# ardaduz/deep-video-mvs

Measured on AMD Instinct MI355X. Metric: depth frames/sec/GPU @ 320x256x64 planes (fusionnet); rel-L1 vs ref, higher is better.
Workload: dtype f32

## Files before the change

deep-video-mvs_amd/csrc/direct_conv.hip:

```cpp
#include <stdlib.h>

#include "dvmvs_device.h"

namespace dvmvs {

typedef float float4v __attribute__((ext_vector_type(4)));

struct DirectConvArgs {
  const float* x;
  const float* packed;
  const float* bias;
  float* dst;
  float* dst_nhwc;
  long long x_batch_stride, dst_batch_stride;
  int B, C_in, C_out, H, W, OH, OW;
  int act;
  int n_groups;
  int packed_groups;
  int n_chunks;
  int tiles_x;
  int vec4;
};

#ifdef DVMVS_SWEEP_TRACE
// ... 343 lines not shown
    }
    const float* xb = x + static_cast<size_t>(b) * x_batch_stride;
#pragma unroll 2
    for (int c = c_lo; c < c_hi; ++c) {
      const float* plane = xb + static_cast<size_t>(c) * HW;
      float v[9];
#pragma unroll
      for (int t = 0; t < 9; ++t) v[t] = in[t] ? plane[off[t]] : 0.0f;
#pragma unroll
      for (int t = 0; t < 9; ++t) sum = fmaf(v[t], w[c * 9 + t], sum);
    }
  }
  s_part[slice][px] = sum;
  __syncthreads();
  if (slice == 0 && p < HW) {
    float total = s_part[0][px];
#pragma unroll
    for (int s = 1; s < SL; ++s) total += s_part[s][px];
    if (bias) total += bias[0];
    dst[static_cast<size_t>(b) * dst_batch_stride + p] = head_activation(total, act, p0, p1);
  }
}

struct DirectConvShape {
  int MW, MT, NT, PW, KS;
};
constexpr DirectConvShape kDcShapes[4] = {{16, 5, 2, 4, 2}, {8, 5, 2, 1, 8}, {16, 5, 1, 1, 8}, {8, 5, 1, 1, 8}};
constexpr int kDcCUs = 256;

inline int direct_conv_choose(int B, int C_in, int C_out, int H, int W, int K, int S) {
  if (B <= 0 || C_in <= 0 || C_out <= 0 || C_out % 16 != 0 || (K != 3 && K != 5) || (S != 1 && S != 2) || H <= 0 || W <= 0) return 0;
  if (S == 2 && (H % 2 != 0 || W % 2 != 0)) return 0;
  const int OH = H / S, OW = W / S;
#if defined(DVMVS_SWEEP_TUNING)
  const char* f = getenv("DVMVS_DC_SHAPE");
  const int forced = f ? atoi(f) : 0;
#else
  const int forced = 0;
#endif
  int best = 0;
  double best_fill = 0.0;
  for (int id = 1; id <= 4; ++id) {
    const DirectConvShape& s = kDcShapes[id - 1];
    const int tile_h = s.PW * (16 / s.MW), tile_w = s.MW * s.MT;
    if (OW % tile_w != 0 || C_out % (16 * s.NT) != 0) continue;
    if (forced == id) return id;
// ... 82 lines not shown
  const int id = direct_conv_choose(B, C_in, C_out, H, W, kernel_size, stride);
  if (id == 0) return DVMVS_EUNSUPPORTED;
  if (kDcShapes[id - 1].NT != n_tile) return DVMVS_EINVAL;
  DirectConvArgs a;
  a.x = x; a.packed = packed; a.bias = bias; a.dst = dst; a.dst_nhwc = dst_nhwc;
  a.B = B; a.C_in = C_in; a.C_out = C_out; a.H = H; a.W = W; a.OH = H / stride; a.OW = W / stride;
  a.x_batch_stride = x_batch_stride ? x_batch_stride : static_cast<long long>(C_in) * H * W;
  a.dst_batch_stride = dst_batch_stride ? dst_batch_stride : static_cast<long long>(C_out) * a.OH * a.OW;
  if (a.x_batch_stride < static_cast<long long>(C_in) * H * W || a.dst_batch_stride < static_cast<long long>(C_out) * a.OH * a.OW) return DVMVS_EINVAL;
  if (W % 4 != 0 || a.x_batch_stride % 4 != 0 || (reinterpret_cast<uintptr_t>(x) & 15) != 0) return DVMVS_EUNSUPPORTED;
  if (static_cast<long long>(C_in + 64) * H * W * 4 >= (1LL << 31)) return DVMVS_EUNSUPPORTED;
  a.act = activation;
  a.n_groups = (C_in + 3) / 4;
  a.packed_groups = dc_packed_groups(C_in);
  a.vec4 = (a.OW % 4 == 0 && (a.OH * a.OW) % 4 == 0 && a.dst_batch_stride % 4 == 0 && (reinterpret_cast<uintptr_t>(dst) & 15) == 0) ? 1 : 0;
  a.n_chunks = 0; a.tiles_x = 0;
  hipStream_t s = static_cast<hipStream_t>(stream);
  if (kernel_size == 3) return stride == 1 ? launch_direct_conv_shape<3, 1>(id, a, s) : launch_direct_conv_shape<3, 2>(id, a, s);
  return stride == 1 ? launch_direct_conv_shape<5, 1>(id, a, s) : launch_direct_conv_shape<5, 2>(id, a, s);
}

extern "C" int dvmvs_conv_head_fwd(const float* x, long long x_batch_stride, const float* weight, const float* bias, float* dst,
                                   long long dst_batch_stride, int B, int C_in, int H, int W, int activation, float p0, float p1, dvmvs_stream_t stream) {
  using namespace dvmvs;
  if (!x || !weight || !dst || B <= 0 || C_in <= 0 || H <= 0 || W <= 0) return DVMVS_EINVAL;
  if (activation < 0 || activation > 3) return DVMVS_EINVAL;
  const long long HW = static_cast<long long>(H) * W;
  if (x_batch_stride == 0) x_batch_stride = HW * C_in;
  if (dst_batch_stride == 0) dst_batch_stride = HW;
  hipStream_t s = static_cast<hipStream_t>(stream);
  if (HW >= 16384) {
    hipLaunchKernelGGL((conv_head_kernel<64>), dim3(static_cast<unsigned int>((HW + 63) / 64), B), dim3(256), 0, s, x, weight, bias, dst, x_batch_stride,
                       dst_batch_stride, C_in, H, W, activation, p0, p1);
  } else {
    hipLaunchKernelGGL((conv_head_kernel<16>), dim3(static_cast<unsigned int>((HW + 15) / 16), B), dim3(256), 0, s, x, weight, bias, dst, x_batch_stride,
                       dst_batch_stride, C_in, H, W, activation, p0, p1);
  }
  return launch_status();
}

#ifdef DVMVS_SWEEP_TRACE
extern "C" int dvmvs_debug_direct_conv_trace(unsigned long long* host, int waves) {
  if (waves > dvmvs::kDcTraceWaves) waves = dvmvs::kDcTraceWaves;
  return static_cast<int>(hipMemcpyFromSymbol(host, HIP_SYMBOL(dvmvs::g_dc_trace), sizeof(unsigned long long) * dvmvs::kDcTraceWords * waves));
}
#endif
```

deep-video-mvs_amd/csrc/frame_ops.hip:

```cpp
#include "dvmvs_device.h"

namespace dvmvs {

template <int ACT>
__device__ inline float apply_act(float v, float p0 = 0.0f, float p1 = 0.0f) {
  if (ACT == 1) return fmaxf(v, 0.0f);
  if (ACT == 2) return 1.0f / (1.0f + expf(-v));
  if (ACT == 3) {
#pragma clang fp contract(off)
    const float s = 1.0f / (1.0f + expf(-v));
    return 1.0f / (p0 * s + p1);
  }
  return v;
}

template <int ACT, bool VEC4, int RES>
__global__ __launch_bounds__(256) void bias_act_kernel(const float* x, float* dst, long long dst_batch_stride, const float* __restrict__ bias,
                                                       const float* __restrict__ residual, int C, int HW, int W, float p0, float p1) {
  const int plane = blockIdx.y;
  const int b = plane / C, c = plane - b * C;
  const float bv = bias ? bias[c] : 0.0f;
  const float* p = x + static_cast<size_t>(plane) * HW;
  float* d = dst + static_cast<size_t>(b) * dst_batch_stride + static_cast<size_t>(c) * HW;
  if (VEC4 && RES != 2) {
    typedef float float4v __attribute__((ext_vector_type(4)));
    const float4v* p4 = reinterpret_cast<const float4v*>(p);
    float4v* d4 = reinterpret_cast<float4v*>(d);
    const float4v* r4 = reinterpret_cast<const float4v*>(residual + (RES == 1 ? static_cast<size_t>(plane) * HW : 0));
    const int n4 = HW / 4;
    for (int i = blockIdx.x * blockDim.x + threadIdx.x; i < n4; i += gridDim.x * blockDim.x) {
      float4v v = p4[i];
#pragma unroll
      for (int e = 0; e < 4; ++e) v[e] = apply_act<ACT>(v[e] + bv, p0, p1);
      if (RES == 1) {
        const float4v r = r4[i];
#pragma unroll
        for (int e = 0; e < 4; ++e) v[e] += r[e];
      }
      d4[i] = v;
    }
  } else {
    const int Wh = W / 2;
    const float* r = RES == 1 ? residual + static_cast<size_t>(plane) * HW
                              : (RES == 2 ? residual + static_cast<size_t>(plane) * (HW / 4) : nullptr);
    for (int i = blockIdx.x * blockDim.x + threadIdx.x; i < HW; i += gridDim.x * blockDim.x) {
      float v = apply_act<ACT>(p[i] + bv, p0, p1);
      if (RES == 1) v += r[i];
      if (RES == 2) {
// ... 13 lines not shown
  const float sh = OH > 1 ? static_cast<float>(H - 1) / static_cast<float>(OH - 1) : 0.0f;
  const float sw = OW > 1 ? static_cast<float>(W - 1) / static_cast<float>(OW - 1) : 0.0f;
  const long long total = static_cast<long long>(planes) * OH * OW;
  for (long long i = blockIdx.x * static_cast<long long>(blockDim.x) + threadIdx.x; i < total;
       i += static_cast<long long>(gridDim.x) * blockDim.x) {
    const int ox = static_cast<int>(i % OW);
    const int oy = static_cast<int>((i / OW) % OH);
    const long long pl = i / (static_cast<long long>(OW) * OH);
    const float fy = sh * static_cast<float>(oy), fx = sw * static_cast<float>(ox);
    const int y0 = static_cast<int>(fy), x0 = static_cast<int>(fx);
    const int y1 = y0 + (y0 < H - 1 ? 1 : 0), x1 = x0 + (x0 < W - 1 ? 1 : 0);
    const float h1 = fy - static_cast<float>(y0), h0 = 1.0f - h1;
    const float w1 = fx - static_cast<float>(x0), w0 = 1.0f - w1;
    const float* p = in + pl * H * W;
    const long long b = pl / C, c = pl - b * C;
    const float bv = (PRE != 0 && pre_bias) ? pre_bias[c] : 0.0f;
    const float v00 = PRE ? apply_act<PRE>(p[y0 * W + x0] + bv) : p[y0 * W + x0], v01 = PRE ? apply_act<PRE>(p[y0 * W + x1] + bv) : p[y0 * W + x1];
    const float v10 = PRE ? apply_act<PRE>(p[y1 * W + x0] + bv) : p[y1 * W + x0], v11 = PRE ? apply_act<PRE>(p[y1 * W + x1] + bv) : p[y1 * W + x1];
    out[b * out_batch_stride + (c * OH + oy) * OW + ox] = h0 * (w0 * v00 + w1 * v01) + h1 * (w0 * v10 + w1 * v11);
  }
}

template <int PRE>
__device__ inline void upsample2x_quads_plane(const float* __restrict__ in, float* __restrict__ out, long long out_batch_stride, const float* __restrict__ pre_bias,
                                              int pl, int C, int H, int W) {
#pragma clang fp contract(off)
  typedef float float4v __attribute__((ext_vector_type(4)));
  const int OH = 2 * H, OW = 2 * W, QW = OW >> 2;
  const float sh = OH > 1 ? static_cast<float>(H - 1) / static_cast<float>(OH - 1) : 0.0f;
  const float sw = OW > 1 ? static_cast<float>(W - 1) / static_cast<float>(OW - 1) : 0.0f;
  const int b = pl / C, c = pl - b * C;
  const float* p = in + static_cast<size_t>(pl) * H * W;
  const float bv = (PRE != 0 && pre_bias) ? pre_bias[c] : 0.0f;
  float* dst = out + static_cast<size_t>(b) * out_batch_stride + static_cast<size_t>(c) * OH * OW;
  for (int q = blockIdx.x * 256 + threadIdx.x; q < OH * QW; q += gridDim.x * 256) {
    const int oy = q / QW, ox = 4 * (q - oy * QW);
    const float fy = sh * static_cast<float>(oy);
    const int y0 = static_cast<int>(fy);
    const int y1 = y0 + (y0 < H - 1 ? 1 : 0);
    const float h1 = fy - static_cast<float>(y0), h0 = 1.0f - h1;
    const float* r0 = p + y0 * W;
    const float* r1 = p + y1 * W;
    float4v v;
#pragma unroll
    for (int e = 0; e < 4; ++e) {
      const float fx = sw * static_cast<float>(ox + e);
      const int x0 = static_cast<int>(fx);
      const int x1 = x0 + (x0 < W - 1 ? 1 : 0);
      const float w1 = fx - static_cast<float>(x0), w0 = 1.0f - w1;
      const float v00 = PRE ? apply_act<PRE>(r0[x0] + bv) : r0[x0], v01 = PRE ? apply_act<PRE>(r0[x1] + bv) : r0[x1];
      const float v10 = PRE ? apply_act<PRE>(r1[x0] + bv) : r1[x0], v11 = PRE ? apply_act<PRE>(r1[x1] + bv) : r1[x1];
      v[e] = h0 * (w0 * v00 + w1 * v01) + h1 * (w0 * v10 + w1 * v11);
    }
    *reinterpret_cast<float4v*>(dst + oy * OW + ox) = v;
  }
}

template <int PRE>
__global__ __launch_bounds__(256) void upsample2x_quads_kernel(const float* __restrict__ in, float* __restrict__ out, long long out_batch_stride,
                                                               const float* __restrict__ pre_bias, int C, int H, int W) {
  upsample2x_quads_plane<PRE>(in, out, out_batch_stride, pre_bias, blockIdx.y, C, H, W);
}

template <int PRE2>
__global__ __launch_bounds__(256) void upsample2x_pair_quads_kernel(const float* __restrict__ in1, float* __restrict__ out1, long long out1_batch_stride, int C1,
                                                                    const float* __restrict__ in2, float* __restrict__ out2, long long out2_batch_stride,
                                                                    const float* __restrict__ pre_bias2, int C2, int planes1, int H, int W) {
  const int pl = blockIdx.y;
  if (pl < planes1) upsample2x_quads_plane<0>(in1, out1, out1_batch_stride, nullptr, pl, C1, H, W);
  else upsample2x_quads_plane<PRE2>(in2, out2, out2_batch_stride, pre_bias2, pl - planes1, C2, H, W);
}

template <int K, int ACT, bool PRE>
__global__ __launch_bounds__(256) void depthwise_conv_kernel(const float* __restrict__ in, const float* __restrict__ weight,
                                                             const float* __restrict__ bias, const float* __restrict__ pre_bias,
                                                             float* __restrict__ out, int C, int H, int W, int OH, int OW, int stride) {
  const int c = blockIdx.y, b = blockIdx.z;
  const float* wk = weight + static_cast<size_t>(c) * K * K;
  const float* src = in + (static_cast<size_t>(b) * C + c) * H * W;
  float* dst = out + (static_cast<size_t>(b) * C + c) * OH * OW;
  const float bv = bias ? bias[c] : 0.0f;
  const float pv = (PRE && pre_bias) ? pre_bias[c] : 0.0f;
  for (int i = blockIdx.x * blockDim.x + threadIdx.x; i < OH * OW; i += gridDim.x * blockDim.x) {
    const int oy = i / OW, ox = i - oy * OW;
    const int y0 = oy * stride - K / 2, x0 = ox * stride - K / 2;
    float acc = 0.0f;
#pragma unroll
    for (int ky = 0; ky < K; ++ky) {
      const int y = y0 + ky;
      const bool yin = y >= 0 && y < H;
#pragma unroll
      for (int kx = 0; kx < K; ++kx) {
        const int x = x0 + kx;
// ... 76 lines not shown
  if (!x || !dst || B <= 0 || C <= 0 || H <= 0 || W <= 0) return DVMVS_EINVAL;
  if (residual_mode < 0 || residual_mode > 2 || (residual_mode != 0 && !residual)) return DVMVS_EINVAL;
  if (dst_batch_stride < static_cast<long long>(C) * H * W) return DVMVS_EINVAL;
  if (residual_mode == 2 && ((H & 1) || (W & 1))) return DVMVS_EUNSUPPORTED;
  if (static_cast<long long>(B) * C > 65535LL) return DVMVS_EUNSUPPORTED;
  hipStream_t s = static_cast<hipStream_t>(stream);
  switch (activation) {
    case 0: return launch_bias_act<0>(x, dst, dst_batch_stride, bias, residual, residual_mode, B, C, H, W, p0, p1, s);
    case 1: return launch_bias_act<1>(x, dst, dst_batch_stride, bias, residual, residual_mode, B, C, H, W, p0, p1, s);
    case 2: return launch_bias_act<2>(x, dst, dst_batch_stride, bias, residual, residual_mode, B, C, H, W, p0, p1, s);
    case 3: return launch_bias_act<3>(x, dst, dst_batch_stride, bias, residual, residual_mode, B, C, H, W, p0, p1, s);
    default: return DVMVS_EINVAL;
  }
}

extern "C" int dvmvs_bias_act_inplace(float* x, const float* bias, const float* residual, int residual_mode, int B, int C, int H,
                                      int W, int activation, dvmvs_stream_t stream) {
  if (activation == 3) return DVMVS_EINVAL;
  return dvmvs_bias_act_fwd(x, x, static_cast<long long>(C) * H * W, bias, residual, residual_mode, B, C, H, W, activation, 0.0f, 0.0f, stream);
}

extern "C" int dvmvs_upsample2x_fwd(const float* in, float* out, long long out_batch_stride, const float* pre_bias, int pre_activation,
                                    int B, int C, int H, int W, dvmvs_stream_t stream) {
  using namespace dvmvs;
  if (!in || !out || B <= 0 || C <= 0 || H <= 0 || W <= 0) return DVMVS_EINVAL;
  if (pre_activation < 0 || pre_activation > 2) return DVMVS_EINVAL;
  if (out_batch_stride == 0) out_batch_stride = static_cast<long long>(C) * H * W * 4;
  if (out_batch_stride < static_cast<long long>(C) * H * W * 4) return DVMVS_EINVAL;
  const long long total = static_cast<long long>(B) * C * H * W * 4;
  long long blocks = (total + 255) / 256;
  if (blocks > 256LL * 16) blocks = 256LL * 16;
  const dim3 grid(static_cast<unsigned>(blocks)), block(256);
  hipStream_t s = static_cast<hipStream_t>(stream);
  if (W % 2 == 0 && (reinterpret_cast<uintptr_t>(out) & 15) == 0 && (out_batch_stride & 3) == 0 && static_cast<long long>(B) * C <= 65535 &&
      static_cast<long long>(H) * W < (1LL << 27)) {
    const int quads = 2 * H * (W / 2);
    const int per_plane = max(1, min((quads + 255) / 256, max(1, 4096 / (B * C))));
    const dim3 qgrid(static_cast<unsigned>(per_plane), static_cast<unsigned>(B * C));
    if (pre_activation == 1) hipLaunchKernelGGL(upsample2x_quads_kernel<1>, qgrid, block, 0, s, in, out, out_batch_stride, pre_bias, C, H, W);
    else if (pre_activation == 2) hipLaunchKernelGGL(upsample2x_quads_kernel<2>, qgrid, block, 0, s, in, out, out_batch_stride, pre_bias, C, H, W);
    else hipLaunchKernelGGL(upsample2x_quads_kernel<0>, qgrid, block, 0, s, in, out, out_batch_stride, pre_bias, C, H, W);
    return launch_status();
  }
  if (pre_activation == 1) hipLaunchKernelGGL(upsample2x_kernel<1>, grid, block, 0, s, in, out, out_batch_stride, pre_bias, B * C, C, H, W);
  else if (pre_activation == 2) hipLaunchKernelGGL(upsample2x_kernel<2>, grid, block, 0, s, in, out, out_batch_stride, pre_bias, B * C, C, H, W);
  else hipLaunchKernelGGL(upsample2x_kernel<0>, grid, block, 0, s, in, out, out_batch_stride, pre_bias, B * C, C, H, W);
  return launch_status();
}

extern "C" int dvmvs_upsample2x_pair_fwd(const float* in1, float* out1, long long out1_batch_stride, int C1, const float* in2, float* out2,
                                         long long out2_batch_stride, const float* pre_bias2, int pre_activation2, int C2, int B, int H, int W,
                                         dvmvs_stream_t stream) {
  using namespace dvmvs;
  if (!in1 || !out1 || !in2 || !out2 || B <= 0 || C1 <= 0 || C2 <= 0 || H <= 0 || W <= 0) return DVMVS_EINVAL;
  if (pre_activation2 < 0 || pre_activation2 > 2) return DVMVS_EINVAL;
  if (out1_batch_stride == 0) out1_batch_stride = static_cast<long long>(C1) * H * W * 4;
  if (out2_batch_stride == 0) out2_batch_stride = static_cast<long long>(C2) * H * W * 4;
  if (out1_batch_stride < static_cast<long long>(C1) * H * W * 4 || out2_batch_stride < static_cast<long long>(C2) * H * W * 4) return DVMVS_EINVAL;
  const long long planes = static_cast<long long>(B) * (C1 + C2);
  const bool quads = W % 2 == 0 && ((reinterpret_cast<uintptr_t>(out1) | reinterpret_cast<uintptr_t>(out2)) & 15) == 0 && ((out1_batch_stride | out2_batch_stride) & 3) == 0 &&
                     planes <= 65535 && static_cast<long long>(H) * W < (1LL << 27);
  if (!quads) {
    const int rc = dvmvs_upsample2x_fwd(in1, out1, out1_batch_stride, nullptr, 0, B, C1, H, W, stream);
    return rc != 0 ? rc : dvmvs_upsample2x_fwd(in2, out2, out2_batch_stride, pre_bias2, pre_activation2, B, C2, H, W, stream);
  }
  const int n_quads = 2 * H * (W / 2);
  const int per_plane = max(1, min((n_quads + 255) / 256, max(1, 4096 / static_cast<int>(planes))));
  const dim3 grid(static_cast<unsigned>(per_plane), static_cast<unsigned>(planes)), block(256);
  hipStream_t s = static_cast<hipStream_t>(stream);
#define DVMVS_UP2(P) hipLaunchKernelGGL(upsample2x_pair_quads_kernel<P>, grid, block, 0, s, in1, out1, out1_batch_stride, C1, in2, out2, out2_batch_stride, pre_bias2, C2, B * C1, H, W)
  if (pre_activation2 == 1) DVMVS_UP2(1); else if (pre_activation2 == 2) DVMVS_UP2(2); else DVMVS_UP2(0);
#undef DVMVS_UP2
  return launch_status();
}

extern "C" int dvmvs_depthwise_conv_fwd(const float* in, const float* weight, const float* bias, const float* pre_bias, int pre_relu,
                                        float* out, int B, int C, int H, int W, int kernel_size, int stride, int activation,
                                        dvmvs_stream_t stream) {
  using namespace dvmvs;
  if (!in || !weight || !out || B <= 0 || C <= 0 || H <= 0 || W <= 0) return DVMVS_EINVAL;
  if ((kernel_size != 3 && kernel_size != 5) || (stride != 1 && stride != 2) || activation < 0 || activation > 2) return DVMVS_EUNSUPPORTED;
  if (C > 65535 || B > 65535) return DVMVS_EUNSUPPORTED;
  const int pad = kernel_size / 2;
  const int OH = (H + 2 * pad - kernel_size) / stride + 1, OW = (W + 2 * pad - kernel_size) / stride + 1;
  hipStream_t s = static_cast<hipStream_t>(stream);
#define DVMVS_DW(K, A) return launch_depthwise<K, A>(in, weight, bias, pre_bias, pre_relu != 0, out, B, C, H, W, OH, OW, stride, s)
  if (kernel_size == 3) {
    if (activation == 0) DVMVS_DW(3, 0);
    if (activation == 1) DVMVS_DW(3, 1);
    DVMVS_DW(3, 2);
  }
  if (activation == 0) DVMVS_DW(5, 0);
  if (activation == 1) DVMVS_DW(5, 1);
  DVMVS_DW(5, 2);
// ... 31 lines not shown
```

deep-video-mvs_amd/dvmvs/hip/_capi.py:

```python
import ctypes
import os
import threading

import torch

_HERE = os.path.dirname(os.path.abspath(__file__))
LIB_PATH = os.environ.get("DVMVS_HIP_LIB", os.path.normpath(os.path.join(_HERE, "..", "..", "lib", "libdvmvs_hip.so")))

ABI_VERSION = 11
MAX_MEASUREMENTS = 8
MAX_DEPTH_LEVELS = 256
LAYOUT_NCHW, LAYOUT_NHWC = 0, 1

_c_fp = ctypes.c_void_p
_c_fpp = ctypes.POINTER(ctypes.c_void_p)
_c_int = ctypes.c_int
_c_dbl = ctypes.c_double
_c_stream = ctypes.c_void_p
_c_f3 = ctypes.POINTER(ctypes.c_float)

SIGNATURES = {
    "dvmvs_abi_version": (_c_int, []),
    "dvmvs_build_arch": (ctypes.c_char_p, []),
    "dvmvs_error_string": (ctypes.c_char_p, [_c_int]),
# ... 21 lines not shown
                                       _c_int, _c_int, _c_int, _c_int, _c_int, _c_int,
                                       _c_dbl, _c_dbl, _c_stream]),
    "dvmvs_hidden_warp_fwd": (_c_int, [_c_fp, _c_fp, _c_fp, _c_fp, _c_fp, _c_int, _c_int, _c_int, _c_int, _c_int, _c_stream]),
    "dvmvs_hidden_warp_bwd": (_c_int, [_c_fp, _c_fp, _c_fp, _c_fp, _c_fp, _c_int, _c_int, _c_int, _c_int, _c_stream]),
    "dvmvs_relative_pose": (_c_int, [_c_fp, _c_fp, _c_fp, _c_int, _c_stream]),
    "dvmvs_lstm_gates_fwd": (_c_int, [_c_fp, _c_fp, _c_fp, _c_fp, _c_int, _c_int, _c_int, _c_int, _c_stream]),
    "dvmvs_lstm_gates_bwd": (_c_int, [_c_fp, _c_fp, _c_fp, _c_fp, _c_fp, _c_fp, _c_int, _c_int, _c_int, _c_int, _c_stream]),
    "dvmvs_lstm_gates_partials_fwd": (_c_int, [_c_fp, _c_int, _c_fp, _c_fp, _c_fp, _c_int, _c_int, _c_int, _c_int, _c_stream]),
    "dvmvs_bottleneck_conv_packed_bytes": (ctypes.c_size_t, [_c_int, _c_int]),
    "dvmvs_bottleneck_conv_pack": (_c_int, [_c_fp, _c_fp, _c_int, _c_int, _c_stream]),
    "dvmvs_bottleneck_conv_splits": (_c_int, [_c_int] * 6),
    "dvmvs_bottleneck_conv_fwd": (_c_int, [_c_fp, _c_fp, _c_fp] + [_c_int] * 6 + [_c_stream]),
    "dvmvs_bottleneck_conv_up2x_fwd": (_c_int, [_c_fp, _c_fp, _c_fp] + [_c_int] * 5 + [_c_stream]),
    "dvmvs_direct_conv_tile": (_c_int, [_c_int] * 7),
    "dvmvs_direct_conv_packed_bytes": (ctypes.c_size_t, [_c_int] * 4),
    "dvmvs_direct_conv_pack": (_c_int, [_c_fp, _c_fp, _c_int, _c_int, _c_int, _c_int, _c_stream]),
    "dvmvs_direct_conv_fwd": (_c_int, [_c_fp, ctypes.c_longlong, _c_fp, _c_int, _c_fp, _c_fp, ctypes.c_longlong] + [_c_int] * 8 + [_c_stream]),
    "dvmvs_direct_conv_dual_fwd": (_c_int, [_c_fp, ctypes.c_longlong, _c_fp, _c_int, _c_fp, _c_fp, ctypes.c_longlong, _c_fp] + [_c_int] * 8 + [_c_stream]),
    "dvmvs_pointwise_conv_supported": (_c_int, [_c_int] * 7),
    "dvmvs_pointwise_conv_packed_bytes": (ctypes.c_size_t, [_c_int] * 2),
    "dvmvs_pointwise_conv_pack": (_c_int, [_c_fp, _c_fp, _c_int, _c_int, _c_stream]),
    "dvmvs_pointwise_conv_fwd": (_c_int, [_c_fp, ctypes.c_longlong, _c_fp, _c_fp, _c_fp, ctypes.c_longlong, _c_int, _c_fp, ctypes.c_longlong] + [_c_int] * 7 + [_c_stream]),
    "dvmvs_conv_head_fwd": (_c_int, [_c_fp, ctypes.c_longlong, _c_fp, _c_fp, _c_fp, ctypes.c_longlong] + [_c_int] * 5 + [ctypes.c_float, ctypes.c_float, _c_stream]),
    "dvmvs_partial_sums_bias_act_fwd": (_c_int, [_c_fp, _c_int, _c_fp, ctypes.c_longlong, _c_fp, _c_int, _c_int, _c_int, _c_int, _c_stream]),
    "dvmvs_depth_reproject_fwd": (_c_int, [_c_fp, _c_fp, _c_fp, _c_fp, _c_fp, _c_fp, _c_int,
                                           _c_int, _c_int, _c_int, _c_stream]),
    "dvmvs_bias_act_fwd": (_c_int, [_c_fp, _c_fp, ctypes.c_longlong, _c_fp, _c_fp, _c_int, _c_int, _c_int, _c_int, _c_int, _c_int,
                                    ctypes.c_float, ctypes.c_float, _c_stream]),
    "dvmvs_bias_act_inplace": (_c_int, [_c_fp, _c_fp, _c_fp, _c_int, _c_int, _c_int, _c_int, _c_int, _c_int, _c_stream]),
    "dvmvs_conv_bias_act_fwd": (_c_int, [_c_fp, _c_fp, _c_fp, _c_fp, ctypes.c_longlong] + [_c_int] * 9 + [_c_stream]),
    "dvmvs_upsample2x_fwd": (_c_int, [_c_fp, _c_fp, ctypes.c_longlong, _c_fp, _c_int, _c_int, _c_int, _c_int, _c_int, _c_stream]),
    "dvmvs_upsample2x_pair_fwd": (_c_int, [_c_fp, _c_fp, ctypes.c_longlong, _c_int, _c_fp, _c_fp, ctypes.c_longlong, _c_fp, _c_int, _c_int, _c_int, _c_int, _c_int, _c_stream]),
    "dvmvs_upsample2x_bwd": (_c_int, [_c_fp, _c_fp, _c_int, _c_int, _c_int, _c_int, _c_stream]),
    "dvmvs_depthwise_conv_bwd_workspace_bytes": (ctypes.c_size_t, [_c_int] * 6),
    "dvmvs_depthwise_conv_bwd": (_c_int, [_c_fp, _c_fp, _c_fp, _c_fp, _c_fp, _c_fp, _c_int, _c_int, _c_int, _c_int, _c_int, _c_int, _c_stream]),
    "dvmvs_depth_reproject_lowres_fwd": (_c_int, [_c_fp, _c_fp, _c_fp, _c_fp, _c_fp, _c_fp, _c_int, _c_int, _c_int, _c_int, _c_stream]),
    "dvmvs_depth_reproject_estimate_fwd": (_c_int, [_c_fp, _c_fp, _c_fp, _c_fp, _c_fp, _c_fp, _c_int, _c_int, _c_int, _c_int, _c_stream]),
    "dvmvs_tsdf_integrate": (_c_int, [_c_fp, _c_fp, _c_fp, _c_int, _c_int, _c_int, ctypes.c_float, ctypes.c_float, ctypes.c_float,
                                      ctypes.c_float, _c_fp, _c_fp, _c_fp, _c_fp, _c_int, _c_int, ctypes.c_float, ctypes.c_float, _c_stream]),
    "dvmvs_marching_cubes_workspace_bytes": (ctypes.c_size_t, [_c_int, _c_int, _c_int]),
    "dvmvs_marching_cubes_count": (_c_int, [_c_fp, _c_int, _c_int, _c_int, ctypes.c_float, _c_fp, ctypes.c_size_t, _c_fp, _c_stream]),
    "dvmvs_marching_cubes_emit": (_c_int, [_c_fp, _c_fp, _c_int, _c_int, _c_int, ctypes.c_float, ctypes.c_float, ctypes.c_float,
                                           ctypes.c_float, ctypes.c_float, _c_fp, _c_fp, _c_fp, _c_fp, _c_fp, ctypes.c_longlong,
                                           ctypes.c_longlong, _c_stream]),
    "dvmvs_depthwise_conv_fwd": (_c_int, [_c_fp, _c_fp, _c_fp, _c_fp, _c_int, _c_fp, _c_int, _c_int, _c_int, _c_int, _c_int, _c_int, _c_int,
                                          _c_stream]),
    "dvmvs_rgb_sweep_fwd": (_c_int, [_c_fp, _c_fpp, _c_fp, _c_fp, _c_fp, _c_int, _c_int, _c_int, _c_int, _c_int, _c_int,
                                     _c_dbl, _c_dbl, _c_int, _c_int, _c_int, _c_stream]),
    "dvmvs_gp_filter_step": (_c_int, [_c_fp, _c_fp, _c_fp, _c_int, _c_dbl, _c_dbl, _c_dbl, _c_dbl, _c_dbl, _c_dbl, _c_int, _c_stream]),
    "dvmvs_dps_volume_fwd": (_c_int, [_c_fp, _c_fp, _c_fp, _c_fp, _c_fp, _c_fp, _c_int, _c_int, _c_int, _c_int, _c_int, _c_dbl, _c_stream]),
    "dvmvs_dps_regress_fwd": (_c_int, [_c_fp, _c_fp, _c_fp, _c_int, _c_int, _c_int, _c_int, _c_int, _c_int, _c_dbl, _c_stream]),
    "dvmvs_preprocess_rgb_fwd": (_c_int, [_c_fp, _c_fp, _c_int, _c_int, _c_int, ctypes.c_longlong, _c_int, _c_int, _c_int, _c_int,
                                          ctypes.c_longlong, _c_dbl, _c_f3, _c_f3, _c_int, _c_stream]),
    "dvmvs_preprocess_depth_fwd": (_c_int, [_c_fp, _c_fp, _c_int, _c_int, _c_int, _c_int, _c_int, _c_int, _c_int, _c_dbl, _c_stream]),
}
# ... 50 lines not shown
```

include/dvmvs_hip.h:

```cpp
#ifndef DVMVS_HIP_H
#define DVMVS_HIP_H

#include <stddef.h>
#include <stdint.h>

#ifdef __cplusplus
extern "C" {
#endif

#define DVMVS_ABI_VERSION 11
#define DVMVS_MAX_MEASUREMENTS 8
#define DVMVS_MAX_DEPTH_LEVELS 256

#define DVMVS_LAYOUT_NCHW 0
#define DVMVS_LAYOUT_NHWC 1

#define DVMVS_EINVAL (-1)
#define DVMVS_EUNSUPPORTED (-2)
#define DVMVS_ELIBRARY (-3)

typedef void* dvmvs_stream_t;

int dvmvs_abi_version(void);
const char* dvmvs_build_arch(void);
// ... 62 lines not shown
size_t dvmvs_bottleneck_conv_packed_bytes(int C_out, int C_in);
int dvmvs_bottleneck_conv_pack(const float* weight, float* packed, int C_out, int C_in, dvmvs_stream_t stream);
int dvmvs_bottleneck_conv_splits(int B, int C_out, int C_in, int H_in, int W_in, int stride);
int dvmvs_bottleneck_conv_fwd(const float* x, const float* packed, float* partials, int B, int C_in, int H_in, int W_in, int C_out,
                              int stride, dvmvs_stream_t stream);
int dvmvs_bottleneck_conv_up2x_fwd(const float* x, const float* packed, float* partials, int B, int C_in, int H_in, int W_in, int C_out,
                                   dvmvs_stream_t stream);
int dvmvs_partial_sums_bias_act_fwd(const float* partials, int n_partials, float* dst, long long dst_batch_stride, const float* bias,
                                    int B, int C, int HW, int activation, dvmvs_stream_t stream);
int dvmvs_lstm_gates_partials_fwd(const float* conv_partials, int n_partials, const float* c_cur, float* h_next, float* c_next,
                                  int B, int hidden, int H, int W, dvmvs_stream_t stream);

int dvmvs_direct_conv_tile(int B, int C_in, int H, int W, int C_out, int kernel_size, int stride);
size_t dvmvs_direct_conv_packed_bytes(int C_out, int C_in, int kernel_size, int n_tile);
int dvmvs_direct_conv_pack(const float* weight, float* packed, int C_out, int C_in, int kernel_size, int n_tile, dvmvs_stream_t stream);
int dvmvs_direct_conv_fwd(const float* x, long long x_batch_stride, const float* packed, int n_tile, const float* bias, float* dst,
                          long long dst_batch_stride, int B, int C_in, int H, int W, int C_out, int kernel_size, int stride, int activation,
                          dvmvs_stream_t stream);
int dvmvs_direct_conv_dual_fwd(const float* x, long long x_batch_stride, const float* packed, int n_tile, const float* bias, float* dst,
                               long long dst_batch_stride, float* dst_nhwc, int B, int C_in, int H, int W, int C_out, int kernel_size, int stride,
                               int activation, dvmvs_stream_t stream);
int dvmvs_conv_head_fwd(const float* x, long long x_batch_stride, const float* weight, const float* bias, float* dst,
                        long long dst_batch_stride, int B, int C_in, int H, int W, int activation, float p0, float p1, dvmvs_stream_t stream);

int dvmvs_pointwise_conv_supported(int B, int C_in, int H, int W, int C_out, int activation, int residual_mode);
size_t dvmvs_pointwise_conv_packed_bytes(int C_out, int C_in);
int dvmvs_pointwise_conv_pack(const float* weight, float* packed, int C_out, int C_in, dvmvs_stream_t stream);
int dvmvs_pointwise_conv_fwd(const float* x, long long x_batch_stride, const float* packed, const float* bias, const float* residual,
                             long long residual_batch_stride, int residual_mode, float* dst, long long dst_batch_stride, int B, int C_in,
                             int H, int W, int C_out, int activation, int splits, dvmvs_stream_t stream);

int dvmvs_depth_reproject_fwd(const float* transformation, const float* previous_depth, const float* full_K,
                              const float* half_K, float* out, float* out_lowres, int lowres_factor,
                              int B, int full_height, int full_width, dvmvs_stream_t stream);
int dvmvs_depth_reproject_lowres_fwd(const float* transformation, const float* previous_depth, const float* full_K,
                                     const float* half_K, float* zbuffer, float* out_lowres, int lowres_factor,
                                     int B, int full_height, int full_width, dvmvs_stream_t stream);

int dvmvs_depth_reproject_estimate_fwd(const float* transformation, const float* previous_depth, const float* full_K,
                                       const float* half_K, float* estimate, float* estimate_to_clear, int lowres_factor,
                                       int B, int full_height, int full_width, dvmvs_stream_t stream);

int dvmvs_bias_act_fwd(const float* x, float* dst, long long dst_batch_stride, const float* bias, const float* residual,
                       int residual_mode, int B, int C, int H, int W, int activation, float p0, float p1, dvmvs_stream_t stream);
int dvmvs_bias_act_inplace(float* x, const float* bias, const float* residual, int residual_mode, int B, int C, int H, int W,
                           int activation, dvmvs_stream_t stream);
int dvmvs_upsample2x_fwd(const float* in, float* out, long long out_batch_stride, const float* pre_bias, int pre_activation,
                         int B, int C, int H, int W, dvmvs_stream_t stream);
int dvmvs_upsample2x_pair_fwd(const float* in1, float* out1, long long out1_batch_stride, int C1, const float* in2, float* out2,
                              long long out2_batch_stride, const float* pre_bias2, int pre_activation2, int C2, int B, int H, int W,
                              dvmvs_stream_t stream);
int dvmvs_conv_bias_act_fwd(const float* x, const float* weight, const float* bias, float* out, long long out_batch_stride,
                            int B, int Cin, int H, int W, int Cout, int K, int stride, int padding, int activation, dvmvs_stream_t stream);
int dvmvs_depthwise_conv_fwd(const float* in, const float* weight, const float* bias, const float* pre_bias, int pre_relu, float* out,
                             int B, int C, int H, int W, int kernel_size, int stride, int activation, dvmvs_stream_t stream);

int dvmvs_tsdf_integrate(float* tsdf_vol, float* weight_vol, float* color_vol, int dim_x, int dim_y, int dim_z,
                         float origin_x, float origin_y, float origin_z, float voxel_size, const float* cam_intr,
                         const float* cam_pose, const float* color_im, const float* depth_im, int im_h, int im_w,
                         float trunc_margin, float obs_weight, dvmvs_stream_t stream);

size_t dvmvs_marching_cubes_workspace_bytes(int X, int Y, int Z);
int dvmvs_marching_cubes_count(const float* vol, int X, int Y, int Z, float level, void* workspace, size_t workspace_bytes,
                               long long* counts_dev, dvmvs_stream_t stream);
int dvmvs_marching_cubes_emit(const float* vol, const float* color_vol, int X, int Y, int Z, float level, float ox, float oy, float oz,
                              float voxel_size, void* workspace, float* verts, float* normals, unsigned char* colors, int* faces,
                              long long V, long long F, dvmvs_stream_t stream);

int dvmvs_rgb_sweep_fwd(const float* image1, const float* const* image2s, const float* Hm, const float* kt, float* out,
                        int B, int M, int C, int H, int W, int D, double min_depth, double max_depth, int Cout,
                        int channel_offset, int copy_image, dvmvs_stream_t stream);
int dvmvs_gp_filter_step(double* state, const float* y, float* z, int N, double a00, double a01, double a10, double a11,
                         double k0, double k1, int reset, dvmvs_stream_t stream);

// ... 16 lines not shown
```

Before: 1410.

## Add register-blocked conv head and two-row bilinear upsample kernels as defaults

```diff
diff --git a/deep-video-mvs_amd/csrc/direct_conv.hip b/deep-video-mvs_amd/csrc/direct_conv.hip
--- a/deep-video-mvs_amd/csrc/direct_conv.hip
+++ b/deep-video-mvs_amd/csrc/direct_conv.hip
@@ -389,6 +389,85 @@
   }
 }
 
+template <int SL, int RUNS, bool VEC>
+__global__ __launch_bounds__(SL * RUNS) void conv_head_runs_kernel(const float* __restrict__ x, const float* __restrict__ w, const float* __restrict__ bias,
+                                                                   float* __restrict__ dst, long long x_batch_stride, long long dst_batch_stride, int C, int H,
+                                                                   int W, int act, float p0, float p1) {
+  constexpr int RUN = 4, CH = 8, NT = SL * RUNS;
+  __shared__ float s_part[SL][RUNS * RUN];
+  const int run = threadIdx.x % RUNS;
+  const int slice = RUNS % 64 == 0 ? __builtin_amdgcn_readfirstlane(threadIdx.x / RUNS) : threadIdx.x / RUNS;
+  const int HW = H * W, rpr = (W + RUN - 1) / RUN;
+  const int b = blockIdx.y;
+  const int g = blockIdx.x * RUNS + run;
+  const int y = g / rpr, x0 = (g - y * rpr) * RUN;
+  const int per = (C + SL - 1) / SL;
+  const int c_lo = slice * per, c_hi = min(C, c_lo + per);
+  float sum[RUN] = {0.0f, 0.0f, 0.0f, 0.0f};
+  if (y < H) {
+    bool rin[3], cin[RUN + 2];
+    int roff[3];
+#pragma unroll
+    for (int r = 0; r < 3; ++r) {
+      const int yy = y + r - 1;
+      rin[r] = yy >= 0 && yy < H;
+      roff[r] = rin[r] ? yy * W + x0 : x0;
+    }
+#pragma unroll
+    for (int j = 0; j < RUN + 2; ++j) cin[j] = x0 + j - 1 >= 0 && x0 + j - 1 < W;
+    const float* xb = x + static_cast<size_t>(b) * x_batch_stride;
+    for (int c0 = c_lo; c0 < c_hi; c0 += CH) {
+      float v[CH][3][RUN + 2];
+#pragma unroll
+      for (int k = 0; k < CH; ++k) {
+        if (c0 + k < c_hi) {
+          const float* plane = xb + static_cast<size_t>(c0 + k) * HW;
+#pragma unroll
+          for (int r = 0; r < 3; ++r) {
+            const float* row = plane + roff[r];
+            if (VEC) {
+              float4v q = {0.0f, 0.0f, 0.0f, 0.0f};
+              if (rin[r]) q = *reinterpret_cast<const float4v*>(row);
+#pragma unroll
+              for (int j = 0; j < RUN; ++j) v[k][r][j + 1] = q[j];
+            } else {
+#pragma unroll
+              for (int j = 1; j <= RUN; ++j) v[k][r][j] = (rin[r] && cin[j]) ? row[j - 1] : 0.0f;
+            }
+            v[k][r][0] = (rin[r] && cin[0]) ? row[-1] : 0.0f;
+            v[k][r][RUN + 1] = (rin[r] && cin[RUN + 1]) ? row[RUN] : 0.0f;
+          }
+        }
+      }
+#pragma unroll
+      for (int k = 0; k < CH; ++k) {
+        if (c0 + k < c_hi) {
+          const float* wc = w + (c0 + k) * 9;
+#pragma unroll
+          for (int e = 0; e < RUN; ++e) {
+#pragma unroll
+            for (int t = 0; t < 9; ++t) sum[e] = fmaf(v[k][t / 3][e + t % 3], wc[t], sum[e]);
+          }
+        }
+      }
+    }
+  }
+#pragma unroll
+  for (int e = 0; e < RUN; ++e) s_part[slice][run * RUN + e] = sum[e];
+  __syncthreads();
+  for (int j = threadIdx.x; j < RUNS * RUN; j += NT) {
+    const int gj = blockIdx.x * RUNS + j / RUN;
+    const int yj = gj / rpr, xj = (gj - yj * rpr) * RUN + j % RUN;
+    if (yj < H && xj < W) {
+      float total = s_part[0][j];
+#pragma unroll
+      for (int s = 1; s < SL; ++s) total += s_part[s][j];
+      if (bias) total += bias[0];
+      dst[static_cast<size_t>(b) * dst_batch_stride + yj * W + xj] = head_activation(total, act, p0, p1);
+    }
+  }
+}
+
 struct DirectConvShape {
   int MW, MT, NT, PW, KS;
 };
@@ -517,20 +596,37 @@
 
 extern "C" int dvmvs_conv_head_fwd(const float* x, long long x_batch_stride, const float* weight, const float* bias, float* dst,
                                    long long dst_batch_stride, int B, int C_in, int H, int W, int activation, float p0, float p1, dvmvs_stream_t stream) {
+  return dvmvs_conv_head_variant_fwd(x, x_batch_stride, weight, bias, dst, dst_batch_stride, B, C_in, H, W, activation, p0, p1, 0, stream);
+}
+
+extern "C" int dvmvs_conv_head_variant_fwd(const float* x, long long x_batch_stride, const float* weight, const float* bias, float* dst,
+                                           long long dst_batch_stride, int B, int C_in, int H, int W, int activation, float p0, float p1, int variant,
+                                           dvmvs_stream_t stream) {
   using namespace dvmvs;
   if (!x || !weight || !dst || B <= 0 || C_in <= 0 || H <= 0 || W <= 0) return DVMVS_EINVAL;
-  if (activation < 0 || activation > 3) return DVMVS_EINVAL;
+  if (activation < 0 || activation > 3 || variant < 0 || variant > 1) return DVMVS_EINVAL;
   const long long HW = static_cast<long long>(H) * W;
   if (x_batch_stride == 0) x_batch_stride = HW * C_in;
   if (dst_batch_stride == 0) dst_batch_stride = HW;
   hipStream_t s = static_cast<hipStream_t>(stream);
-  if (HW >= 16384) {
-    hipLaunchKernelGGL((conv_head_kernel<64>), dim3(static_cast<unsigned int>((HW + 63) / 64), B), dim3(256), 0, s, x, weight, bias, dst, x_batch_stride,
-                       dst_batch_stride, C_in, H, W, activation, p0, p1);
-  } else {
-    hipLaunchKernelGGL((conv_head_kernel<16>), dim3(static_cast<unsigned int>((HW + 15) / 16), B), dim3(256), 0, s, x, weight, bias, dst, x_batch_stride,
-                       dst_batch_stride, C_in, H, W, activation, p0, p1);
-  }
+  const bool large = HW >= 16384;
+  if (variant == 1) {
+    if (large) {
+      hipLaunchKernelGGL((conv_head_kernel<64>), dim3(static_cast<unsigned int>((HW + 63) / 64), B), dim3(256), 0, s, x, weight, bias, dst, x_batch_stride,
+                         dst_batch_stride, C_in, H, W, activation, p0, p1);
+    } else {
+      hipLaunchKernelGGL((conv_head_kernel<16>), dim3(static_cast<unsigned int>((HW + 15) / 16), B), dim3(256), 0, s, x, weight, bias, dst, x_batch_stride,
+                         dst_batch_stride, C_in, H, W, activation, p0, p1);
+    }
+    return launch_status();
+  }
+  const long long runs = static_cast<long long>(H) * ((W + 3) / 4);
+  const bool vec = W % 4 == 0 && x_batch_stride % 4 == 0 && (reinterpret_cast<uintptr_t>(x) & 15) == 0;
+#define DVMVS_HEAD(SL, RUNS, V) hipLaunchKernelGGL((conv_head_runs_kernel<SL, RUNS, V>), dim3(static_cast<unsigned int>((runs + RUNS - 1) / RUNS), B), dim3(SL * RUNS), \
+                                                   0, s, x, weight, bias, dst, x_batch_stride, dst_batch_stride, C_in, H, W, activation, p0, p1)
+  if (large) { if (vec) DVMVS_HEAD(4, 64, true); else DVMVS_HEAD(4, 64, false); }
+  else { if (vec) DVMVS_HEAD(16, 4, true); else DVMVS_HEAD(16, 4, false); }
+#undef DVMVS_HEAD
   return launch_status();
 }
 
diff --git a/deep-video-mvs_amd/csrc/frame_ops.hip b/deep-video-mvs_amd/csrc/frame_ops.hip
--- a/deep-video-mvs_amd/csrc/frame_ops.hip
+++ b/deep-video-mvs_amd/csrc/frame_ops.hip
@@ -1,6 +1,8 @@
 #include "dvmvs_device.h"
 
 namespace dvmvs {
+
+typedef float float4v __attribute__((ext_vector_type(4)));
 
 template <int ACT>
 __device__ inline float apply_act(float v, float p0 = 0.0f, float p1 = 0.0f) {
@@ -23,7 +25,6 @@
   const float* p = x + static_cast<size_t>(plane) * HW;
   float* d = dst + static_cast<size_t>(b) * dst_batch_stride + static_cast<size_t>(c) * HW;
   if (VEC4 && RES != 2) {
-    typedef float float4v __attribute__((ext_vector_type(4)));
     const float4v* p4 = reinterpret_cast<const float4v*>(p);
     float4v* d4 = reinterpret_cast<float4v*>(d);
     const float4v* r4 = reinterpret_cast<const float4v*>(residual + (RES == 1 ? static_cast<size_t>(plane) * HW : 0));
@@ -83,10 +84,34 @@
 }
 
 template <int PRE>
+__device__ inline float4v upsample2x_row_quad(const float* __restrict__ p, float bv, float sh, float sw, int oy, int ox, int H, int W) {
+#pragma clang fp contract(off)
+  const float fy = sh * static_cast<float>(oy);
+  const int y0 = static_cast<int>(fy);
+  const int y1 = y0 + (y0 < H - 1 ? 1 : 0);
+  const float h1 = fy - static_cast<float>(y0), h0 = 1.0f - h1;
+  const float* r0 = p + y0 * W;
+  const float* r1 = p + y1 * W;
+  float4v v;
+#pragma unroll
+  for (int e = 0; e < 4; ++e) {
+    const float fx = sw * static_cast<float>(ox + e);
+    const int x0 = static_cast<int>(fx);
+    const int x1 = x0 + (x0 < W - 1 ? 1 : 0);
+    const float w1 = fx - static_cast<float>(x0), w0 = 1.0f - w1;
+    const float v00 = PRE ? apply_act<PRE>(r0[x0] + bv) : r0[x0], v01 = PRE ? apply_act<PRE>(r0[x1] + bv) : r0[x1];
+    const float v10 = PRE ? apply_act<PRE>(r1[x0] + bv) : r1[x0], v11 = PRE ? apply_act<PRE>(r1[x1] + bv) : r1[x1];
+    v[e] = h0 * (w0 * v00 + w1 * v01) + h1 * (w0 * v10 + w1 * v11);
+  }
+  return v;
+}
+
+__device__ inline float pick4(const float (&v)[4], int k) { return k == 0 ? v[0] : (k == 1 ? v[1] : (k == 2 ? v[2] : v[3])); }
+
+template <int PRE, bool ROWS>
 __device__ inline void upsample2x_quads_plane(const float* __restrict__ in, float* __restrict__ out, long long out_batch_stride, const float* __restrict__ pre_bias,
                                               int pl, int C, int H, int W) {
 #pragma clang fp contract(off)
-  typedef float float4v __attribute__((ext_vector_type(4)));
   const int OH = 2 * H, OW = 2 * W, QW = OW >> 2;
   const float sh = OH > 1 ? static_cast<float>(H - 1) / static_cast<float>(OH - 1) : 0.0f;
   const float sw = OW > 1 ? static_cast<float>(W - 1) / static_cast<float>(OW - 1) : 0.0f;
@@ -94,42 +119,83 @@
   const float* p = in + static_cast<size_t>(pl) * H * W;
   const float bv = (PRE != 0 && pre_bias) ? pre_bias[c] : 0.0f;
   float* dst = out + static_cast<size_t>(b) * out_batch_stride + static_cast<size_t>(c) * OH * OW;
-  for (int q = blockIdx.x * 256 + threadIdx.x; q < OH * QW; q += gridDim.x * 256) {
-    const int oy = q / QW, ox = 4 * (q - oy * QW);
-    const float fy = sh * static_cast<float>(oy);
-    const int y0 = static_cast<int>(fy);
-    const int y1 = y0 + (y0 < H - 1 ? 1 : 0);
-    const float h1 = fy - static_cast<float>(y0), h0 = 1.0f - h1;
-    const float* r0 = p + y0 * W;
-    const float* r1 = p + y1 * W;
-    float4v v;
+  if (ROWS) {
+    for (int q = blockIdx.x * 256 + threadIdx.x; q < OH * QW; q += gridDim.x * 256) {
+      const int oy = q / QW, ox = 4 * (q - oy * QW);
+      *reinterpret_cast<float4v*>(dst + oy * OW + ox) = upsample2x_row_quad<PRE>(p, bv, sh, sw, oy, ox, H, W);
+    }
+    return;
+  }
+  for (int q = blockIdx.x * 256 + threadIdx.x; q < H * QW; q += gridDim.x * 256) {
+    const int k = q / QW, oy = 2 * k, ox = 4 * (q - k * QW);
+    int y0[2], y1[2], x0[4], x1[4];
+    float h0[2], h1[2], w0[4], w1[4];
+#pragma unroll
+    for (int a = 0; a < 2; ++a) {
+      const float fy = sh * static_cast<float>(oy + a);
+      y0[a] = static_cast<int>(fy);
+      y1[a] = y0[a] + (y0[a] < H - 1 ? 1 : 0);
+      h1[a] = fy - static_cast<float>(y0[a]);
+      h0[a] = 1.0f - h1[a];
+    }
 #pragma unroll
     for (int e = 0; e < 4; ++e) {
       const float fx = sw * static_cast<float>(ox + e);
-      const int x0 = static_cast<int>(fx);
-      const int x1 = x0 + (x0 < W - 1 ? 1 : 0);
-      const float w1 = fx - static_cast<float>(x0), w0 = 1.0f - w1;
-      const float v00 = PRE ? apply_act<PRE>(r0[x0] + bv) : r0[x0], v01 = PRE ? apply_act<PRE>(r0[x1] + bv) : r0[x1];
-      const float v10 = PRE ? apply_act<PRE>(r1[x0] + bv) : r1[x0], v11 = PRE ? apply_act<PRE>(r1[x1] + bv) : r1[x1];
-      v[e] = h0 * (w0 * v00 + w1 * v01) + h1 * (w0 * v10 + w1 * v11);
-    }
-    *reinterpret_cast<float4v*>(dst + oy * OW + ox) = v;
-  }
-}
-
-template <int PRE>
+      x0[e] = static_cast<int>(fx);
+      x1[e] = x0[e] + (x0[e] < W - 1 ? 1 : 0);
+      w1[e] = fx - static_cast<float>(x0[e]);
+      w0[e] = 1.0f - w1[e];
+    }
+    const int yb = y0[0], xb = x0[0];
+    bool fits = y0[1] >= yb && y0[1] <= yb + 1;
+#pragma unroll
+    for (int e = 1; e < 4; ++e) fits = fits && x0[e] >= xb && x0[e] <= xb + 2;
+    if (!fits) {
+#pragma unroll
+      for (int a = 0; a < 2; ++a) *reinterpret_cast<float4v*>(dst + (oy + a) * OW + ox) = upsample2x_row_quad<PRE>(p, bv, sh, sw, oy + a, ox, H, W);
+      continue;
+    }
+    float t[3][4];
+#pragma unroll
+    for (int i = 0; i < 3; ++i) {
+      const float* r = p + min(yb + i, H - 1) * W;
+      float v[4];
+#pragma unroll
+      for (int j = 0; j < 4; ++j) {
+        const float s = r[min(xb + j, W - 1)];
+        v[j] = PRE ? apply_act<PRE>(s + bv) : s;
+      }
+#pragma unroll
+      for (int e = 0; e < 4; ++e) t[i][e] = w0[e] * pick4(v, x0[e] - xb) + w1[e] * pick4(v, x1[e] - xb);
+    }
+#pragma unroll
+    for (int a = 0; a < 2; ++a) {
+      const int d0 = y0[a] - yb, d1 = y1[a] - yb;
+      float4v o;
+#pragma unroll
+      for (int e = 0; e < 4; ++e) {
+        const float top = d0 == 0 ? t[0][e] : t[1][e];
+        const float bottom = d1 == 0 ? t[0][e] : (d1 == 1 ? t[1][e] : t[2][e]);
+        o[e] = h0[a] * top + h1[a] * bottom;
+      }
+      *reinterpret_cast<float4v*>(dst + (oy + a) * OW + ox) = o;
+    }
+  }
+}
+
+template <int PRE, bool ROWS>
 __global__ __launch_bounds__(256) void upsample2x_quads_kernel(const float* __restrict__ in, float* __restrict__ out, long long out_batch_stride,
                                                                const float* __restrict__ pre_bias, int C, int H, int W) {
-  upsample2x_quads_plane<PRE>(in, out, out_batch_stride, pre_bias, blockIdx.y, C, H, W);
-}
-
-template <int PRE2>
+  upsample2x_quads_plane<PRE, ROWS>(in, out, out_batch_stride, pre_bias, blockIdx.y, C, H, W);
+}
+
+template <int PRE2, bool ROWS>
 __global__ __launch_bounds__(256) void upsample2x_pair_quads_kernel(const float* __restrict__ in1, float* __restrict__ out1, long long out1_batch_stride, int C1,
                                                                     const float* __restrict__ in2, float* __restrict__ out2, long long out2_batch_stride,
                                                                     const float* __restrict__ pre_bias2, int C2, int planes1, int H, int W) {
   const int pl = blockIdx.y;
-  if (pl < planes1) upsample2x_quads_plane<0>(in1, out1, out1_batch_stride, nullptr, pl, C1, H, W);
-  else upsample2x_quads_plane<PRE2>(in2, out2, out2_batch_stride, pre_bias2, pl - planes1, C2, H, W);
+  if (pl < planes1) upsample2x_quads_plane<0, ROWS>(in1, out1, out1_batch_stride, nullptr, pl, C1, H, W);
+  else upsample2x_quads_plane<PRE2, ROWS>(in2, out2, out2_batch_stride, pre_bias2, pl - planes1, C2, H, W);
 }
 
 template <int K, int ACT, bool PRE>
@@ -252,9 +318,14 @@
 
 extern "C" int dvmvs_upsample2x_fwd(const float* in, float* out, long long out_batch_stride, const float* pre_bias, int pre_activation,
                                     int B, int C, int H, int W, dvmvs_stream_t stream) {
+  return dvmvs_upsample2x_variant_fwd(in, out, out_batch_stride, pre_bias, pre_activation, B, C, H, W, 0, stream);
+}
+
+extern "C" int dvmvs_upsample2x_variant_fwd(const float* in, float* out, long long out_batch_stride, const float* pre_bias, int pre_activation,
+                                            int B, int C, int H, int W, int variant, dvmvs_stream_t stream) {
   using namespace dvmvs;
   if (!in || !out || B <= 0 || C <= 0 || H <= 0 || W <= 0) return DVMVS_EINVAL;
-  if (pre_activation < 0 || pre_activation > 2) return DVMVS_EINVAL;
+  if (pre_activation < 0 || pre_activation > 2 || variant < 0 || variant > 1) return DVMVS_EINVAL;
   if (out_batch_stride == 0) out_batch_stride = static_cast<long long>(C) * H * W * 4;
   if (out_batch_stride < static_cast<long long>(C) * H * W * 4) return DVMVS_EINVAL;
   const long long total = static_cast<long long>(B) * C * H * W * 4;
@@ -264,12 +335,13 @@
   hipStream_t s = static_cast<hipStream_t>(stream);
   if (W % 2 == 0 && (reinterpret_cast<uintptr_t>(out) & 15) == 0 && (out_batch_stride & 3) == 0 && static_cast<long long>(B) * C <= 65535 &&
       static_cast<long long>(H) * W < (1LL << 27)) {
-    const int quads = 2 * H * (W / 2);
-    const int per_plane = max(1, min((quads + 255) / 256, max(1, 4096 / (B * C))));
+    const int items = (variant == 1 ? 2 : 1) * H * (W / 2);
+    const int per_plane = max(1, min((items + 255) / 256, max(1, 4096 / (B * C))));
     const dim3 qgrid(static_cast<unsigned>(per_plane), static_cast<unsigned>(B * C));
-    if (pre_activation == 1) hipLaunchKernelGGL(upsample2x_quads_kernel<1>, qgrid, block, 0, s, in, out, out_batch_stride, pre_bias, C, H, W);
-    else if (pre_activation == 2) hipLaunchKernelGGL(upsample2x_quads_kernel<2>, qgrid, block, 0, s, in, out, out_batch_stride, pre_bias, C, H, W);
-    else hipLaunchKernelGGL(upsample2x_quads_kernel<0>, qgrid, block, 0, s, in, out, out_batch_stride, pre_bias, C, H, W);
+#define DVMVS_UP1(P, R) hipLaunchKernelGGL((upsample2x_quads_kernel<P, R>), qgrid, block, 0, s, in, out, out_batch_stride, pre_bias, C, H, W)
+    if (variant == 1) { if (pre_activation == 1) DVMVS_UP1(1, true); else if (pre_activation == 2) DVMVS_UP1(2, true); else DVMVS_UP1(0, true); }
+    else { if (pre_activation == 1) DVMVS_UP1(1, false); else if (pre_activation == 2) DVMVS_UP1(2, false); else DVMVS_UP1(0, false); }
+#undef DVMVS_UP1
     return launch_status();
   }
   if (pre_activation == 1) hipLaunchKernelGGL(upsample2x_kernel<1>, grid, block, 0, s, in, out, out_batch_stride, pre_bias, B * C, C, H, W);
@@ -281,9 +353,15 @@
 extern "C" int dvmvs_upsample2x_pair_fwd(const float* in1, float* out1, long long out1_batch_stride, int C1, const float* in2, float* out2,
                                          long long out2_batch_stride, const float* pre_bias2, int pre_activation2, int C2, int B, int H, int W,
                                          dvmvs_stream_t stream) {
+  return dvmvs_upsample2x_pair_variant_fwd(in1, out1, out1_batch_stride, C1, in2, out2, out2_batch_stride, pre_bias2, pre_activation2, C2, B, H, W, 0, stream);
+}
+
+extern "C" int dvmvs_upsample2x_pair_variant_fwd(const float* in1, float* out1, long long out1_batch_stride, int C1, const float* in2, float* out2,
+                                                 long long out2_batch_stride, const float* pre_bias2, int pre_activation2, int C2, int B, int H, int W,
+                                                 int variant, dvmvs_stream_t stream) {
   using namespace dvmvs;
   if (!in1 || !out1 || !in2 || !out2 || B <= 0 || C1 <= 0 || C2 <= 0 || H <= 0 || W <= 0) return DVMVS_EINVAL;
-  if (pre_activation2 < 0 || pre_activation2 > 2) return DVMVS_EINVAL;
+  if (pre_activation2 < 0 || pre_activation2 > 2 || variant < 0 || variant > 1) return DVMVS_EINVAL;
   if (out1_batch_stride == 0) out1_batch_stride = static_cast<long long>(C1) * H * W * 4;
   if (out2_batch_stride == 0) out2_batch_stride = static_cast<long long>(C2) * H * W * 4;
   if (out1_batch_stride < static_cast<long long>(C1) * H * W * 4 || out2_batch_stride < static_cast<long long>(C2) * H * W * 4) return DVMVS_EINVAL;
@@ -291,15 +369,16 @@
   const bool quads = W % 2 == 0 && ((reinterpret_cast<uintptr_t>(out1) | reinterpret_cast<uintptr_t>(out2)) & 15) == 0 && ((out1_batch_stride | out2_batch_stride) & 3) == 0 &&
                      planes <= 65535 && static_cast<long long>(H) * W < (1LL << 27);
   if (!quads) {
-    const int rc = dvmvs_upsample2x_fwd(in1, out1, out1_batch_stride, nullptr, 0, B, C1, H, W, stream);
-    return rc != 0 ? rc : dvmvs_upsample2x_fwd(in2, out2, out2_batch_stride, pre_bias2, pre_activation2, B, C2, H, W, stream);
-  }
-  const int n_quads = 2 * H * (W / 2);
-  const int per_plane = max(1, min((n_quads + 255) / 256, max(1, 4096 / static_cast<int>(planes))));
+    const int rc = dvmvs_upsample2x_variant_fwd(in1, out1, out1_batch_stride, nullptr, 0, B, C1, H, W, variant, stream);
+    return rc != 0 ? rc : dvmvs_upsample2x_variant_fwd(in2, out2, out2_batch_stride, pre_bias2, pre_activation2, B, C2, H, W, variant, stream);
+  }
+  const int items = (variant == 1 ? 2 : 1) * H * (W / 2);
+  const int per_plane = max(1, min((items + 255) / 256, max(1, 4096 / static_cast<int>(planes))));
   const dim3 grid(static_cast<unsigned>(per_plane), static_cast<unsigned>(planes)), block(256);
   hipStream_t s = static_cast<hipStream_t>(stream);
-#define DVMVS_UP2(P) hipLaunchKernelGGL(upsample2x_pair_quads_kernel<P>, grid, block, 0, s, in1, out1, out1_batch_stride, C1, in2, out2, out2_batch_stride, pre_bias2, C2, B * C1, H, W)
-  if (pre_activation2 == 1) DVMVS_UP2(1); else if (pre_activation2 == 2) DVMVS_UP2(2); else DVMVS_UP2(0);
+#define DVMVS_UP2(P, R) hipLaunchKernelGGL((upsample2x_pair_quads_kernel<P, R>), grid, block, 0, s, in1, out1, out1_batch_stride, C1, in2, out2, out2_batch_stride, pre_bias2, C2, B * C1, H, W)
+  if (variant == 1) { if (pre_activation2 == 1) DVMVS_UP2(1, true); else if (pre_activation2 == 2) DVMVS_UP2(2, true); else DVMVS_UP2(0, true); }
+  else { if (pre_activation2 == 1) DVMVS_UP2(1, false); else if (pre_activation2 == 2) DVMVS_UP2(2, false); else DVMVS_UP2(0, false); }
 #undef DVMVS_UP2
   return launch_status();
 }
diff --git a/deep-video-mvs_amd/dvmvs/hip/_capi.py b/deep-video-mvs_amd/dvmvs/hip/_capi.py
--- a/deep-video-mvs_amd/dvmvs/hip/_capi.py
+++ b/deep-video-mvs_amd/dvmvs/hip/_capi.py
@@ -67,6 +67,7 @@
     "dvmvs_pointwise_conv_pack": (_c_int, [_c_fp, _c_fp, _c_int, _c_int, _c_stream]),
     "dvmvs_pointwise_conv_fwd": (_c_int, [_c_fp, ctypes.c_longlong, _c_fp, _c_fp, _c_fp, ctypes.c_longlong, _c_int, _c_fp, ctypes.c_longlong] + [_c_int] * 7 + [_c_stream]),
     "dvmvs_conv_head_fwd": (_c_int, [_c_fp, ctypes.c_longlong, _c_fp, _c_fp, _c_fp, ctypes.c_longlong] + [_c_int] * 5 + [ctypes.c_float, ctypes.c_float, _c_stream]),
+    "dvmvs_conv_head_variant_fwd": (_c_int, [_c_fp, ctypes.c_longlong, _c_fp, _c_fp, _c_fp, ctypes.c_longlong] + [_c_int] * 5 + [ctypes.c_float, ctypes.c_float, _c_int, _c_stream]),
     "dvmvs_partial_sums_bias_act_fwd": (_c_int, [_c_fp, _c_int, _c_fp, ctypes.c_longlong, _c_fp, _c_int, _c_int, _c_int, _c_int, _c_stream]),
     "dvmvs_depth_reproject_fwd": (_c_int, [_c_fp, _c_fp, _c_fp, _c_fp, _c_fp, _c_fp, _c_int,
                                            _c_int, _c_int, _c_int, _c_stream]),
@@ -76,6 +77,8 @@
     "dvmvs_conv_bias_act_fwd": (_c_int, [_c_fp, _c_fp, _c_fp, _c_fp, ctypes.c_longlong] + [_c_int] * 9 + [_c_stream]),
     "dvmvs_upsample2x_fwd": (_c_int, [_c_fp, _c_fp, ctypes.c_longlong, _c_fp, _c_int, _c_int, _c_int, _c_int, _c_int, _c_stream]),
     "dvmvs_upsample2x_pair_fwd": (_c_int, [_c_fp, _c_fp, ctypes.c_longlong, _c_int, _c_fp, _c_fp, ctypes.c_longlong, _c_fp, _c_int, _c_int, _c_int, _c_int, _c_int, _c_stream]),
+    "dvmvs_upsample2x_variant_fwd": (_c_int, [_c_fp, _c_fp, ctypes.c_longlong, _c_fp, _c_int, _c_int, _c_int, _c_int, _c_int, _c_int, _c_stream]),
+    "dvmvs_upsample2x_pair_variant_fwd": (_c_int, [_c_fp, _c_fp, ctypes.c_longlong, _c_int, _c_fp, _c_fp, ctypes.c_longlong, _c_fp, _c_int, _c_int, _c_int, _c_int, _c_int, _c_int, _c_stream]),
     "dvmvs_upsample2x_bwd": (_c_int, [_c_fp, _c_fp, _c_int, _c_int, _c_int, _c_int, _c_stream]),
     "dvmvs_depthwise_conv_bwd_workspace_bytes": (ctypes.c_size_t, [_c_int] * 6),
     "dvmvs_depthwise_conv_bwd": (_c_int, [_c_fp, _c_fp, _c_fp, _c_fp, _c_fp, _c_fp, _c_int, _c_int, _c_int, _c_int, _c_int, _c_int, _c_stream]),
diff --git a/include/dvmvs_hip.h b/include/dvmvs_hip.h
--- a/include/dvmvs_hip.h
+++ b/include/dvmvs_hip.h
@@ -108,6 +108,9 @@
                                int activation, dvmvs_stream_t stream);
 int dvmvs_conv_head_fwd(const float* x, long long x_batch_stride, const float* weight, const float* bias, float* dst,
                         long long dst_batch_stride, int B, int C_in, int H, int W, int activation, float p0, float p1, dvmvs_stream_t stream);
+int dvmvs_conv_head_variant_fwd(const float* x, long long x_batch_stride, const float* weight, const float* bias, float* dst,
+                                long long dst_batch_stride, int B, int C_in, int H, int W, int activation, float p0, float p1, int variant,
+                                dvmvs_stream_t stream);
 
 int dvmvs_pointwise_conv_supported(int B, int C_in, int H, int W, int C_out, int activation, int residual_mode);
 size_t dvmvs_pointwise_conv_packed_bytes(int C_out, int C_in);
@@ -136,6 +139,11 @@
 int dvmvs_upsample2x_pair_fwd(const float* in1, float* out1, long long out1_batch_stride, int C1, const float* in2, float* out2,
                               long long out2_batch_stride, const float* pre_bias2, int pre_activation2, int C2, int B, int H, int W,
                               dvmvs_stream_t stream);
+int dvmvs_upsample2x_variant_fwd(const float* in, float* out, long long out_batch_stride, const float* pre_bias, int pre_activation,
+                                 int B, int C, int H, int W, int variant, dvmvs_stream_t stream);
+int dvmvs_upsample2x_pair_variant_fwd(const float* in1, float* out1, long long out1_batch_stride, int C1, const float* in2, float* out2,
+                                      long long out2_batch_stride, const float* pre_bias2, int pre_activation2, int C2, int B, int H, int W,
+                                      int variant, dvmvs_stream_t stream);
 int dvmvs_conv_bias_act_fwd(const float* x, const float* weight, const float* bias, float* out, long long out_batch_stride,
                             int B, int Cin, int H, int W, int Cout, int K, int stride, int padding, int activation, dvmvs_stream_t stream);
 int dvmvs_depthwise_conv_fwd(const float* in, const float* weight, const float* bias, const float* pre_bias, int pre_relu, float* out,
```

Result: slower. 1395 (-1.1%).
